# IRVLab/so_dso_place_recognition

Measured on AMD Instinct MI355X. Metric: queries/sec over 100k-signature DB (SC 20x60, z-score fusion, top-1), higher is better.
Workload: dtype f16x2 (fp32 carried as f16 hi + lo, fp32 accumulate); binary intensity channel: one f16 product per term, rounded to its exact integer count; 1 GPU; sc_match_100k; db_signatures=100000, descriptor=SC 20x60 x 2 channels, mask_width=0, k=1, db_rows_per_gpu=100000

## Files before the change

### so_dso_place_recognition_amd/csrc/sc_pack.hip

```cpp
#include <cstdlib>
#include <cstring>

#include "kernels.hpp"

namespace pr {
namespace {

constexpr int SC_PACK_FEW = 8;

template <typename T>
__global__ __launch_bounds__(256) void sc_pack_kernel(const T* __restrict__ sig, int rows, int role,
                                                       float* __restrict__ packed, int groups,
                                                       const double* __restrict__ tw, int* __restrict__ flags,
                                                       int* __restrict__ bad) {
  __shared__ double x[1200];
  __shared__ double red[256];
  __shared__ double tws[120];
  const int tid = threadIdx.x;
  const int row = blockIdx.x >> 1, ch = blockIdx.x & 1;
  const T* src = sig + (size_t)row * 2400 + ch * 1200;
  double part = 0.0;
  for (int i = tid; i < 1200; i += 256) {
    double v = (double)src[i];
    x[i] = v;
    part += v * v;
  }
  if (tid < 120) tws[tid] = tw[tid];
  red[tid] = part;
  __syncthreads();
  for (int s = 128; s > 0; s >>= 1) {
    if (tid < s) red[tid] += red[tid + s];
    __syncthreads();
  }
  const double nr = sqrt(red[0]);
  const bool isbad = !(nr > 0.0) || !(nr < __builtin_inf());
  if (tid == 0) { bad[2 * row + ch] = isbad ? (1 << ch) : 0; if (isbad) atomicOr(flags, 1); }
  for (int i = tid; i < 1200; i += 256) x[i] = isbad ? 0.0 : x[i] / nr;
  __syncthreads();
  const double scale = 0.12909944487358055;
  for (int o = tid; o < SC_NF * 40; o += 256) {
    const int f = o / 40, rem = o - f * 40, ring = rem >> 1, im = rem & 1;
    double acc = 0.0;
    int t = 0;
    for (int s = 0; s < 60; s++) {
      const double w = im ? -tws[60 + t] : tws[t];
      acc += x[s * 20 + ring] * w;
      t += f;
      if (t >= 60) t -= 60;
    }
    const float val = (float)(acc * scale);
    const int s4 = ring >> 2, k = ring & 3;
    size_t dst;
    if (role == 0) {
      const int g = row >> 3, e = row & 7;
      const int lane = (k << 4) | (im << 3) | e;
      dst = ((size_t)ch * groups + g) * SC_QIMG + (size_t)sc_fpos(f) * 320 + s4 * 64 + lane;
    } else {
      const int g = row >> 4, j = row & 15;
      const int lane = (k << 4) | j;
      const size_t base = ((size_t)ch * groups + g) * SC_DIMG + (size_t)sc_fpos(f) * SC_DSTEP;
      dst = (s4 < 4) ? base + im * 256 + lane * 4 + s4 : base + 512 + lane * 2 + im;
    }
    packed[dst] = val;
  }
}


template <typename T>
__global__ __launch_bounds__(320) void sc_pack_h_kernel(const T* __restrict__ sig, int rows, int role,
                                                         unsigned short* __restrict__ packed, int groups,
                                                         const double* __restrict__ tw, int* __restrict__ flags,
                                                         int* __restrict__ bad) {
  __shared__ double x[1200];
  __shared__ double red[320];
  __shared__ double tws[120];
  const int tid = threadIdx.x;
  const int row = blockIdx.x >> 1, ch = blockIdx.x & 1;
  const T* src = sig + (size_t)row * 2400 + ch * 1200;
  double part = 0.0;
  for (int i = tid; i < 1200; i += 320) {
    double v = (double)src[i];
    x[i] = v;
    part += v * v;
  }
  if (tid < 120) tws[tid] = tw[tid];
  red[tid] = part;
  __syncthreads();
  if (tid < 64) red[tid] += red[tid + 256];
  __syncthreads();
  for (int s = 128; s > 0; s >>= 1) {
    if (tid < s) red[tid] += red[tid + s];
    __syncthreads();
  }
  const double nr = sqrt(red[0]);
  const bool isbad = !(nr > 0.0) || !(nr < __builtin_inf());
  if (tid == 0) { bad[2 * row + ch] = isbad ? (1 << ch) : 0; if (isbad) atomicOr(flags, 1); }
  for (int i = tid; i < 1200; i += 320) x[i] = isbad ? 0.0 : x[i] / nr;
  __syncthreads();
  const double scale = 0.12909944487358055 * (role == 0 ? 256.0 : 128.0);
  {
    const int o = tid;
    const int f = o / 20, ring = o - f * 20;
    double ce = 0.0, co = 0.0, se = 0.0, so = 0.0;
    int t = 0;
#pragma unroll 3
    for (int s2 = 0; s2 < 60; s2 += 2) {
      const double x0 = x[s2 * 20 + ring];
      ce += x0 * tws[t];
      se += x0 * tws[60 + t];
      t += f; if (t >= 60) t -= 60;
      const double x1 = x[(s2 + 1) * 20 + ring];
      co += x1 * tws[t];
      so += x1 * tws[60 + t];
      t += f; if (t >= 60) t -= 60;
    }
    auto put = [&](double val, int ff, int im) {
      const _Float16 hi = (_Float16)val;
      const _Float16 lo = (_Float16)(val - (double)hi);
      size_t bh, bl;
      if (role == 0) {
        const int g = row >> 3, rr = (im << 3) | (row & 7);
        const size_t base = ((size_t)ch * groups + g) * SCH_QIMG + (size_t)ff * SCH_QBLK + rr * 80 + (rr >= 8 ? 8 : 0);
        bh = base + ring * 2;
        bl = base + sch_qlo_byte(ring);
      } else {
        const int g = row >> 4, j = row & 15;
        const size_t base = ((size_t)ch * groups + g) * SCH_DIMG + (size_t)ff * SCH_DFREQ + (size_t)im * 2 * SCH_DTILE +
                            (((ring >> 3) << 4) | j) * 16 + (ring & 7) * 2;
        bh = base;
        bl = base + SCH_DTILE;
        if (ring >= 16) packed[(bl + 8) >> 1] = __builtin_bit_cast(unsigned short, hi);
      }
      packed[bh >> 1] = __builtin_bit_cast(unsigned short, hi);
      packed[bl >> 1] = __builtin_bit_cast(unsigned short, lo);
    };
    put((ce + co) * scale, f, 0);
    put(-(se + so) * scale, f, 1);
    if (f != 15) {
      put((ce - co) * scale, 30 - f, 0);
      put((se - so) * scale, 30 - f, 1);
    }
  }
}

template <typename T, int ROLE, bool LO>
__global__ __launch_bounds__(320) void sc_pack_h_col_kernel(const T* __restrict__ sig, int rows,
                                                             unsigned short* __restrict__ packed, int groups,
                                                             const double* __restrict__ tw, int* __restrict__ flags,
                                                             int* __restrict__ bad, float* __restrict__ binfo, int* __restrict__ bstat) {
  constexpr int SL = ROLE == 0 ? (LO ? SCH_QBLK : SCF_QBLK) : (LO ? SCH_DFREQ : SCF_DFREQ);
  constexpr int NG = ROLE == 0 ? 2 : 1;
  constexpr int IMGB = ROLE == 0 ? (LO ? SCH_QIMG : SCF_QIMG) : (LO ? SCH_DIMG : SCF_DIMG);
  constexpr int QROW = LO ? 80 : 40;
  __shared__ __attribute__((aligned(16))) char img[NG * 8 * SL];
  __shared__ double part[16 * 20];
  __shared__ int bnz[LO ? 320 : 1];
  __shared__ float epart[LO ? 320 : 1];
  const int tid = threadIdx.x, lrow = tid / 20, ring = tid - 20 * lrow;
  const int xcd = blockIdx.x & 7, idx = blockIdx.x >> 3;
  const int fb = idx & 3, ch = (idx >> 2) & 1, blk = (idx >> 3) * 8 + xcd;
  if (blk * 16 >= rows) return;
  const int row = blk * 16 + lrow;
  const bool valid = row < rows;
  for (int i = tid; i < NG * 8 * SL / 8; i += 320) reinterpret_cast<unsigned long long*>(img)[i] = 0ull;
  const T* src = sig + (size_t)(valid ? row : 0) * 2400 + ch * 1200 + ring;
  double ce[4] = {0, 0, 0, 0}, co[4] = {0, 0, 0, 0}, se[4] = {0, 0, 0, 0}, so[4] = {0, 0, 0, 0};
  double nsq = 0.0;
  const bool do_eps = LO && binfo != nullptr && ch == 1, do_bin = do_eps && fb == 0;
  int nz = 0;
  double vmn = __builtin_inf(), vmx = -__builtin_inf();
  float e2 = 0.f;
  const double* twc = tw + 120 + (size_t)fb * 60 * 8;
#ifndef SCP_AHEAD
#define SCP_AHEAD 2
#endif
  constexpr int XR = SCP_AHEAD + 1;
  static_assert(15 % XR == 0, "the ring size must divide the 15 rounds");
  T xq[XR][4];
#pragma unroll
  for (int r = 0; r < SCP_AHEAD; r++)
#pragma unroll
    for (int k = 0; k < 4; k++) xq[r][k] = src[(r * 4 + k) * 20];
#pragma unroll XR
  for (int it = 0; it < 15; it++) {
    if (it + SCP_AHEAD < 15) {
#pragma unroll
      for (int k = 0; k < 4; k++) xq[(it + SCP_AHEAD) % XR][k] = src[((it + SCP_AHEAD) * 4 + k) * 20];
    }
    int tz = 0;
    asm volatile("" : "+s"(tz), "+v"(ce[0]), "+v"(ce[1]), "+v"(ce[2]), "+v"(ce[3]), "+v"(co[0]), "+v"(co[1]), "+v"(co[2]), "+v"(co[3]),
                      "+v"(se[0]), "+v"(se[1]), "+v"(se[2]), "+v"(se[3]), "+v"(so[0]), "+v"(so[1]), "+v"(so[2]), "+v"(so[3]));
    const double* tp = twc + it * 32 + tz;
#pragma unroll
    for (int h = 0; h < 2; h++) {
      const double x0 = (double)xq[it % XR][2 * h], x1 = (double)xq[it % XR][2 * h + 1];
      nsq += x0 * x0;
      nsq += x1 * x1;
      if (do_bin) {
        if (x0 != 0.0) { nz++; vmn = fmin(vmn, x0); vmx = fmax(vmx, x0); }
        if (x1 != 0.0) { nz++; vmn = fmin(vmn, x1); vmx = fmax(vmx, x1); }
      }
#pragma unroll
      for (int j = 0; j < 4; j++) {
        ce[j] += x0 * tp[h * 16 + 2 * j];
        se[j] += x0 * tp[h * 16 + 2 * j + 1];
        co[j] += x1 * tp[h * 16 + 8 + 2 * j];
        so[j] += x1 * tp[h * 16 + 8 + 2 * j + 1];
      }
    }
  }
  part[tid] = nsq;
  if (LO && do_bin) bnz[tid] = (nz == 0 || (vmn == vmx && vmn > 0.0)) ? nz : -1;
  __syncthreads();
  double n2 = 0.0;
#pragma unroll
  for (int r = 0; r < 20; r++) n2 += part[lrow * 20 + r];
  const double nr = sqrt(n2);
  const bool isbad = !(nr > 0.0) || !(nr < __builtin_inf());
  if (valid && ring == 0 && fb == 0) { bad[2 * row + ch] = isbad ? (1 << ch) : 0; if (isbad) atomicOr(flags, 1); }
  const int srow = blk * 16 + tid;
  bool sbad = true;
  if (LO && do_eps && tid < 16) {
    double n2t = 0.0;
#pragma unroll
    for (int r = 0; r < 20; r++) n2t += part[tid * 20 + r];
    const double nrt = sqrt(n2t);
    sbad = srow >= rows || !(nrt > 0.0) || !(nrt < __builtin_inf());
  }
  if (LO && do_bin) {
    __syncthreads();
    part[tid] = vmx;
    __syncthreads();
    if (tid < 16) {
      int ones = 0;
      bool binary = true;
      double a = -__builtin_inf();
      for (int r = 0; r < 20; r++) {
        const int c = bnz[tid * 20 + r];
        const double v = part[tid * 20 + r];
        if (c < 0) binary = false;
        if (c > 0) { ones += c; if (a == -__builtin_inf()) a = v; else if (v != a) binary = false; }
      }
      binary = binary && ones > 0;
      float s1 = 1.f, rs = 1.f;
      if (!sbad && binary) { s1 = (float)sqrt((double)ones); rs = (float)(1.0 / sqrt((double)ones)); }
      if (srow < rows) { binfo[2 * srow] = s1; binfo[2 * srow + 1] = rs; }
      int mo = (!sbad && binary) ? ones : 0, nb = (!sbad && !binary) ? 1 : 0;
#pragma unroll
      for (int o = 8; o > 0; o >>= 1) { mo = max(mo, __shfl_xor(mo, o)); nb |= __shfl_xor(nb, o); }
      if (tid == 0) { bstat[SC_BSTAT_INTS + 6 * blk] = nb; bstat[SC_BSTAT_INTS + 6 * blk + 1] = mo; }
    }
  }
  const double sc = isbad ? 0.0 : 0.12909944487358055 * (ROLE == 0 ? 256.0 : 128.0) / nr;
  auto put = [&](double val, int slice, int im) {
    if (isbad) val = 0.0;
    float vf = (float)val;
    asm volatile("" : "+v"(vf));
    const _Float16 hi = (_Float16)vf;
    float rf = (float)(val - (double)hi);
    asm volatile("" : "+v"(rf));
    const _Float16 lo = (_Float16)rf;
    int bh, bl;
    if (ROLE == 0) {
      const int rr = (im << 3) | (lrow & 7);
      bh = ((lrow >> 3) * 8 + slice) * SL + rr * QROW + ((LO && rr >= 8) ? 8 : 0) + ring * 2;
      bl = bh - ring * 2 + sch_qlo_byte(ring);
    } else {
      bh = slice * SL + im * (LO ? 2 : 1) * SCH_DTILE + (((ring >> 3) << 4) | lrow) * 16 + (ring & 7) * 2;
      bl = bh + SCH_DTILE;
      if (LO && ring >= 16) *reinterpret_cast<_Float16*>(img + bl + 8) = hi;
    }
    *reinterpret_cast<_Float16*>(img + bh) = hi;
    if (LO) *reinterpret_cast<_Float16*>(img + bl) = lo;
    if (LO) {
      const bool edge = (fb == 0 && (slice & 3) == 0);
      e2 = __builtin_fmaf(edge ? rf : 2.f * rf, rf, e2);
    }
  };
  if (valid) {
#pragma unroll
    for (int j = 0; j < 4; j++) {
      put((ce[j] + co[j]) * sc, j, 0);
      put(-(se[j] + so[j]) * sc, j, 1);
      if (4 * fb + j != 15) {
        put((ce[j] - co[j]) * sc, 4 + j, 0);
        put((se[j] - so[j]) * sc, 4 + j, 1);
      }
    }
  }
  if (LO && do_eps) epart[tid] = e2;
  __syncthreads();
  if (LO && do_eps && tid < 16) {
    float e = 0.f;
    for (int r = 0; r < 20; r++) e += epart[tid * 20 + r];
    if (sbad) e = 0.f;
#pragma unroll
    for (int o = 8; o > 0; o >>= 1) e = fmaxf(e, __shfl_xor(e, o));
    const int eb = __float_as_int(e * (ROLE == 0 ? 0x1p-16f : 0x1p-14f) * (1.f + 0x1p-10f));
    if (tid == 0) bstat[SC_BSTAT_INTS + 6 * blk + 2 + fb] = eb;
  }
  constexpr int W = SL / 8;
  for (int i = tid; i < NG * 8 * W; i += 320) {
    const int sl = i / W, wd = i - sl * W, gg = sl >> 3, k = sl & 7;
    const int f = k < 4 ? 4 * fb + k : 30 - 4 * fb - (k - 4);
    if (k >= 4 && f == 15) continue;
    const int g = NG * blk + gg;
    if (g >= groups) continue;
    reinterpret_cast<unsigned long long*>(reinterpret_cast<char*>(packed) + ((size_t)ch * groups + g) * IMGB + (size_t)f * SL)[wd] =
        reinterpret_cast<const unsigned long long*>(img)[i];
  }
}

__device__ __forceinline__ double wave_sum(double v) {
#pragma unroll
  for (int o = 32; o > 0; o >>= 1) v += __shfl_xor(v, o);
  return v;
}
template <typename T, int ROLE, bool LO>
__global__ __launch_bounds__(320) void sc_pack_h_few_kernel(const T* __restrict__ sig, int rows, unsigned short* __restrict__ packed, int groups,
                                                             const double* __restrict__ tw, int* __restrict__ flags, int* __restrict__ bad,
                                                             float* __restrict__ binfo, int* __restrict__ bstat,
                                                             int row0 ) {
  constexpr int SL = ROLE == 0 ? (LO ? SCH_QBLK : SCF_QBLK) : (LO ? SCH_DFREQ : SCF_DFREQ);
  constexpr int IMGB = ROLE == 0 ? (LO ? SCH_QIMG : SCF_QIMG) : (LO ? SCH_DIMG : SCF_DIMG);
  constexpr int QROW = LO ? 80 : 40;
  __shared__ double x[1200];
  __shared__ double tws[120];
  __shared__ double part[20];
  __shared__ double wred[5][3];
  const int tid = threadIdx.x, f = tid / 20, ring = tid - 20 * f;
  const int row = row0 + (blockIdx.x >> 1), ch = blockIdx.x & 1;
  const T* src = sig + (size_t)(blockIdx.x >> 1) * 2400 + ch * 1200;
  const bool do_bin = LO && binfo != nullptr && ch == 1;
  double bz = 0.0, bmn_ = __builtin_inf(), bmx_ = -__builtin_inf();
  for (int i = tid; i < 1200; i += 320) {
    const double v = (double)src[i];
    x[i] = v;
    if (do_bin && v != 0.0) { bz += 1.0; bmn_ = fmin(bmn_, v); bmx_ = fmax(bmx_, v); }
  }
  if (do_bin) {
#pragma unroll
    for (int o = 32; o > 0; o >>= 1) { bz += __shfl_xor(bz, o); bmn_ = fmin(bmn_, __shfl_xor(bmn_, o)); bmx_ = fmax(bmx_, __shfl_xor(bmx_, o)); }
    if ((tid & 63) == 0) { wred[tid >> 6][0] = bz; wred[tid >> 6][1] = bmn_; wred[tid >> 6][2] = bmx_; }
  }
  if (tid < 120) tws[tid] = tw[tid];
  __syncthreads();
  double ce = 0.0, co = 0.0, se = 0.0, so = 0.0, nsq = 0.0;
  int t = 0;
#pragma unroll 1
  for (int s2 = 0; s2 < 60; s2 += 2) {
    const double x0 = x[s2 * 20 + ring], x1 = x[(s2 + 1) * 20 + ring];
    nsq += x0 * x0;
    nsq += x1 * x1;
    ce += x0 * tws[t];
    se += x0 * tws[60 + t];
    t += f; if (t >= 60) t -= 60;
    co += x1 * tws[t];
    so += x1 * tws[60 + t];
    t += f; if (t >= 60) t -= 60;
  }
  if (f == 0) part[ring] = nsq;
  __syncthreads();
  double n2 = 0.0;
#pragma unroll
  for (int r = 0; r < 20; r++) n2 += part[r];
  const double nr = sqrt(n2);
  const bool isbad = !(nr > 0.0) || !(nr < __builtin_inf());
  if (tid == 0) { bad[2 * row + ch] = isbad ? (1 << ch) : 0; if (isbad) atomicOr(flags, 1); }
  if (do_bin && tid == 0) {
    double ones = 0.0, mn = __builtin_inf(), mx = -__builtin_inf();
    for (int w5 = 0; w5 < 5; w5++) { ones += wred[w5][0]; mn = fmin(mn, wred[w5][1]); mx = fmax(mx, wred[w5][2]); }
    const bool binary = ones > 0.0 && mn == mx && mn > 0.0;
    float s = 1.f, rs = 1.f;
    if (!isbad && binary) { s = (float)sqrt(ones); rs = (float)(1.0 / sqrt(ones)); atomicMax(bstat + 1, (int)ones); }
    if (!isbad && !binary) atomicOr(bstat, 1);
    binfo[2 * row] = s; binfo[2 * row + 1] = rs;
  }
  const double sc = isbad ? 0.0 : 0.12909944487358055 * (ROLE == 0 ? 256.0 : 128.0) / nr;
  char* out = reinterpret_cast<char*>(packed);
  double e2 = 0.0;
  auto put = [&](double val, int ff, int im) {
    if (isbad) val = 0.0;
    float vf = (float)val;
    asm volatile("" : "+v"(vf));
    const _Float16 hi = (_Float16)vf;
    float rf = (float)(val - (double)hi);
    asm volatile("" : "+v"(rf));
    const _Float16 lo = (_Float16)rf;
    if (do_bin) {
      const double r = (val - (double)hi) * (ROLE == 0 ? 0x1p-8 : 0x1p-7);
      e2 += ((ff == 0 || ff == 30) ? 1.0 : 2.0) * r * r;
    }
    size_t bh;
    if (ROLE == 0) {
      const int g = row >> 3, rr = (im << 3) | (row & 7);
      bh = ((size_t)ch * groups + g) * IMGB + (size_t)ff * SL + rr * QROW + ((LO && rr >= 8) ? 8 : 0) + ring * 2;
      *reinterpret_cast<_Float16*>(out + bh) = hi;
      if (LO) *reinterpret_cast<_Float16*>(out + bh - ring * 2 + sch_qlo_byte(ring)) = lo;
    } else {
      const int g = row >> 4, j = row & 15;
      bh = ((size_t)ch * groups + g) * IMGB + (size_t)ff * SL + (size_t)im * (LO ? 2 : 1) * SCH_DTILE + (((ring >> 3) << 4) | j) * 16 + (ring & 7) * 2;
      *reinterpret_cast<_Float16*>(out + bh) = hi;
      if (LO) *reinterpret_cast<_Float16*>(out + bh + SCH_DTILE) = lo;
      if (LO && ring >= 16) *reinterpret_cast<_Float16*>(out + bh + SCH_DTILE + 8) = hi;
    }
  };
  put((ce + co) * sc, f, 0);
  put(-(se + so) * sc, f, 1);
  if (f != 15) {
    put((ce - co) * sc, 30 - f, 0);
    put((se - so) * sc, 30 - f, 1);
  }
  if (do_bin) {
    e2 = wave_sum(e2);
    __syncthreads();
    if ((tid & 63) == 0) wred[tid >> 6][0] = e2;
    __syncthreads();
    if (tid == 0 && !isbad) {
      double e = 0.0;
      for (int w5 = 0; w5 < 5; w5++) e += wred[w5][0];
      atomicMax(bstat + 2, __float_as_int((float)(e * (1.0 + 0x1p-20))));
    }
  }
}

__global__ __launch_bounds__(256) void sc_bstat_finalize_kernel(int* __restrict__ bstat, int nblk) {
  __shared__ int red[6][256];
  int v[6] = {0, 0, 0, 0, 0, 0};
  for (int b = threadIdx.x; b < nblk; b += 256) {
    const int* w = bstat + SC_BSTAT_INTS + 6 * b;
    v[0] |= w[0];
#pragma unroll
    for (int i = 1; i < 6; i++) v[i] = max(v[i], w[i]);
  }
#pragma unroll
  for (int i = 0; i < 6; i++) red[i][threadIdx.x] = v[i];
  __syncthreads();
  for (int s2 = 128; s2 > 0; s2 >>= 1) {
    if ((int)threadIdx.x < s2) {
      red[0][threadIdx.x] |= red[0][threadIdx.x + s2];
#pragma unroll
      for (int i = 1; i < 6; i++) red[i][threadIdx.x] = max(red[i][threadIdx.x], red[i][threadIdx.x + s2]);
    }
    __syncthreads();
  }
  if (threadIdx.x < 6) bstat[threadIdx.x] = red[threadIdx.x][0];
}

template <typename T, int ROLE, bool LO = true>
void launch_pack_col(hipStream_t st, const T* sig, int rows, unsigned short* packed, int groups, const double* tw, int* flags, int* bad,
                     float* binfo = nullptr, int* bstat = nullptr) {
  if (rows <= SC_PACK_FEW) {
    hipLaunchKernelGGL((sc_pack_h_few_kernel<T, ROLE, LO>), dim3((unsigned)rows * 2), dim3(320), 0, st, sig, rows, packed, groups, tw, flags, bad,
                       binfo, bstat, 0);
    return;
  }
  hipLaunchKernelGGL((sc_pack_h_col_kernel<T, ROLE, LO>), dim3((unsigned)(((rows + 15) / 16 + 7) / 8) * 64), dim3(320), 0, st, sig, rows, packed,
                     groups, tw, flags, bad, binfo, bstat);
  if (LO && bstat) hipLaunchKernelGGL(sc_bstat_finalize_kernel, dim3(1), dim3(256), 0, st, bstat, (rows + 15) / 16);
}

__global__ __launch_bounds__(256) void zero_ints_kernel(int* __restrict__ p, int n) {
  const int i = blockIdx.x * 256 + threadIdx.x;
  if (i < n) p[i] = 0;
}

__global__ __launch_bounds__(256) void fill_ints_kernel(int* __restrict__ p, int n, int v) {
  const int i = blockIdx.x * 256 + threadIdx.x;
  if (i < n) p[i] = v;
}

}

void launch_zero_ints(hipStream_t st, int* p, int n) {
  if (n > 0) hipLaunchKernelGGL(zero_ints_kernel, dim3((n + 255) / 256), dim3(256), 0, st, p, n);
}
void launch_fill_ints(hipStream_t st, int* p, int n, int v) {
  if (n > 0) hipLaunchKernelGGL(fill_ints_kernel, dim3((n + 255) / 256), dim3(256), 0, st, p, n, v);
}

void launch_sc_pack_h(hipStream_t st, const void* sig, int dtype, int rows, int role, void* packed, int groups,
                      const double* twiddle, int* flags, int* bad, int single, float* binfo, int* bstat) {
  if (rows <= 0) return;
  if (single) {
    if (dtype == 0 && role == 0) launch_pack_col<double, 0, false>(st, (const double*)sig, rows, (unsigned short*)packed, groups, twiddle, flags, bad);
    else if (dtype == 0) launch_pack_col<double, 1, false>(st, (const double*)sig, rows, (unsigned short*)packed, groups, twiddle, flags, bad);
    else if (role == 0) launch_pack_col<float, 0, false>(st, (const float*)sig, rows, (unsigned short*)packed, groups, twiddle, flags, bad);
    else launch_pack_col<float, 1, false>(st, (const float*)sig, rows, (unsigned short*)packed, groups, twiddle, flags, bad);
    return;
  }
  static const bool valu = getenv("PR_SC_PACK") && !strcmp(getenv("PR_SC_PACK"), "valu");
  if (valu && bstat) hipLaunchKernelGGL(fill_ints_kernel, dim3(1), dim3(256), 0, st, bstat, 1, 1);
  if (valu && dtype == 0)
    hipLaunchKernelGGL(sc_pack_h_kernel<double>, dim3(rows * 2), dim3(320), 0, st, (const double*)sig, rows, role,
                       (unsigned short*)packed, groups, twiddle, flags, bad);
  else if (valu)
    hipLaunchKernelGGL(sc_pack_h_kernel<float>, dim3(rows * 2), dim3(320), 0, st, (const float*)sig, rows, role,
                       (unsigned short*)packed, groups, twiddle, flags, bad);
  else if (dtype == 0 && role == 0) launch_pack_col<double, 0>(st, (const double*)sig, rows, (unsigned short*)packed, groups, twiddle, flags, bad, binfo, bstat);
  else if (dtype == 0) launch_pack_col<double, 1>(st, (const double*)sig, rows, (unsigned short*)packed, groups, twiddle, flags, bad, binfo, bstat);
  else if (role == 0) launch_pack_col<float, 0>(st, (const float*)sig, rows, (unsigned short*)packed, groups, twiddle, flags, bad, binfo, bstat);
  else launch_pack_col<float, 1>(st, (const float*)sig, rows, (unsigned short*)packed, groups, twiddle, flags, bad, binfo, bstat);
}

void launch_sc_pack_h_rows(hipStream_t st, const void* sig, int dtype, int rows, int row0, void* packed, int groups, const double* twiddle,
                           int* flags, int* bad, int single, float* binfo, int* bstat) {
  if (rows <= 0) return;
  unsigned short* pk = (unsigned short*)packed;
  const dim3 grid((unsigned)rows * 2), blk(320);
  if (single) {
    if (dtype == 0) hipLaunchKernelGGL((sc_pack_h_few_kernel<double, 1, false>), grid, blk, 0, st, (const double*)sig, rows, pk, groups, twiddle, flags, bad, nullptr, nullptr, row0);
    else hipLaunchKernelGGL((sc_pack_h_few_kernel<float, 1, false>), grid, blk, 0, st, (const float*)sig, rows, pk, groups, twiddle, flags, bad, nullptr, nullptr, row0);
  } else {
    if (dtype == 0) hipLaunchKernelGGL((sc_pack_h_few_kernel<double, 1, true>), grid, blk, 0, st, (const double*)sig, rows, pk, groups, twiddle, flags, bad, binfo, bstat, row0);
    else hipLaunchKernelGGL((sc_pack_h_few_kernel<float, 1, true>), grid, blk, 0, st, (const float*)sig, rows, pk, groups, twiddle, flags, bad, binfo, bstat, row0);
  }
}

void launch_sc_pack(hipStream_t st, const void* sig, int dtype, int rows, int role, float* packed, int groups,
                    const double* twiddle, int* flags, int* bad) {
  if (rows <= 0) return;
  if (dtype == 0)
    hipLaunchKernelGGL(sc_pack_kernel<double>, dim3(rows * 2), dim3(256), 0, st, (const double*)sig, rows, role,
                       packed, groups, twiddle, flags, bad);
  else
    hipLaunchKernelGGL(sc_pack_kernel<float>, dim3(rows * 2), dim3(256), 0, st, (const float*)sig, rows, role,
                       packed, groups, twiddle, flags, bad);
}

}
```

Baseline: 138,600 queries/s.

## Replace direct DFT in SC packing with factored real FFT-60

The column pack kernel now computes each 60-point ring DFT with a factored real FFT (radix-4 by 15, with the 15-point part split as 3 by 5) held in registers per thread, instead of a twiddle-table direct DFT where each thread produced one frequency. One block now handles all 31 frequencies of 16 rows and writes them out in four staged slices, so the grid shrinks and the per-element multiply-adds drop from O(N^2) to roughly O(N log N). The few-row kernel also uses the FFT, on 20 threads. The old kernel stays behind a PR_SC_PACK=dense env switch. In exchange, the roughly 60-double register arrays raise register pressure, and the rounding differs from the direct sum, which could change the hi/lo split bits.

```diff
diff --git a/so_dso_place_recognition_amd/csrc/sc_pack.hip b/so_dso_place_recognition_amd/csrc/sc_pack.hip
--- a/so_dso_place_recognition_amd/csrc/sc_pack.hip
+++ b/so_dso_place_recognition_amd/csrc/sc_pack.hip
@@ -144,7 +144,7 @@
 }
 
 template <typename T, int ROLE, bool LO>
-__global__ __launch_bounds__(320) void sc_pack_h_col_kernel(const T* __restrict__ sig, int rows,
+__global__ __launch_bounds__(320) void sc_pack_h_col_dense_kernel(const T* __restrict__ sig, int rows,
                                                              unsigned short* __restrict__ packed, int groups,
                                                              const double* __restrict__ tw, int* __restrict__ flags,
                                                              int* __restrict__ bad, float* __restrict__ binfo, int* __restrict__ bstat) {
@@ -311,6 +311,251 @@
   }
 }
 
+struct ScR5 { double a0, a1, b1, a2, b2; };
+__device__ __forceinline__ ScR5 sc_rdft5(double r0, double r1, double r2, double r3, double r4) {
+#pragma clang fp contract(off)
+  constexpr double C1 = 0.30901699437494742410, C2 = -0.80901699437494742410;
+  constexpr double S1 = 0.95105651629515357212, S2 = 0.58778525229247312917;
+  const double s1 = r1 + r4, s2 = r2 + r3, d1 = r1 - r4, d2 = r2 - r3;
+  ScR5 o;
+  o.a0 = r0 + (s1 + s2);
+  o.a1 = __builtin_fma(C2, s2, __builtin_fma(C1, s1, r0));
+  o.a2 = __builtin_fma(C1, s2, __builtin_fma(C2, s1, r0));
+  o.b1 = __builtin_fma(S2, d2, S1 * d1);
+  o.b2 = __builtin_fma(-S1, d2, S2 * d1);
+  return o;
+}
+template <int ST>
+__device__ __forceinline__ void sc_rdft15(const double* z, double* re, double* im) {
+#pragma clang fp contract(off)
+  constexpr double S3 = 0.86602540378443864676;
+  double r0[5], p[5], q[5];
+#pragma unroll
+  for (int b = 0; b < 5; b++) {
+    const double z0 = z[ST * ((3 * b) % 15)], z1 = z[ST * ((5 + 3 * b) % 15)], z2 = z[ST * ((10 + 3 * b) % 15)];
+    const double s = z1 + z2;
+    r0[b] = z0 + s;
+    p[b] = __builtin_fma(-0.5, s, z0);
+    q[b] = S3 * (z2 - z1);
+  }
+  const ScR5 v0 = sc_rdft5(r0[0], r0[1], r0[2], r0[3], r0[4]);
+  const ScR5 vp = sc_rdft5(p[0], p[1], p[2], p[3], p[4]);
+  const ScR5 vq = sc_rdft5(q[0], q[1], q[2], q[3], q[4]);
+  re[0] = v0.a0;          im[0] = 0.0;
+  re[1] = vp.a1 + vq.b1;  im[1] = vq.a1 - vp.b1;
+  re[2] = vp.a2 - vq.b2;  im[2] = -(vq.a2 + vp.b2);
+  re[3] = v0.a2;          im[3] = v0.b2;
+  re[4] = vp.a1 - vq.b1;  im[4] = vq.a1 + vp.b1;
+  re[5] = vp.a0;          im[5] = -vq.a0;
+  re[6] = v0.a1;          im[6] = -v0.b1;
+  re[7] = vp.a2 + vq.b2;  im[7] = vq.a2 - vp.b2;
+}
+__device__ __forceinline__ void sc_rdft60(const double* x, double* re, double* im) {
+#pragma clang fp contract(off)
+  double z[60];
+#pragma unroll
+  for (int m = 0; m < 15; m++) {
+    const double a = x[(4 * m) % 60], b = x[(15 + 4 * m) % 60], c = x[(30 + 4 * m) % 60], d = x[(45 + 4 * m) % 60];
+    const double ac = a + c, bd = b + d;
+    z[4 * m] = ac + bd;
+    z[4 * m + 1] = ac - bd;
+    z[4 * m + 2] = a - c;
+    z[4 * m + 3] = b - d;
+  }
+  double u0r[8], u0i[8], u2r[8], u2i[8], ar[8], ai[8], br[8], bi[8];
+  sc_rdft15<4>(z, u0r, u0i);
+  sc_rdft15<4>(z + 1, u2r, u2i);
+  sc_rdft15<4>(z + 2, ar, ai);
+  sc_rdft15<4>(z + 3, br, bi);
+#pragma unroll
+  for (int k = 0; k <= 30; k++) {
+    const int k15 = k % 15, kk = k15 <= 7 ? k15 : 15 - k15;
+    const double cj = k15 <= 7 ? 1.0 : -1.0;
+    switch (k & 3) {
+      case 0: re[k] = u0r[kk]; im[k] = cj * u0i[kk]; break;
+      case 2: re[k] = u2r[kk]; im[k] = cj * u2i[kk]; break;
+      case 1: re[k] = ar[kk] + cj * bi[kk]; im[k] = cj * ai[kk] - br[kk]; break;
+      default: re[k] = ar[kk] - cj * bi[kk]; im[k] = cj * ai[kk] + br[kk]; break;
+    }
+  }
+}
+
+__device__ __forceinline__ double sc_row_sq(const double* x) {
+  double nsq = 0.0;
+#pragma unroll
+  for (int s = 0; s < 60; s++) nsq = __builtin_fma(x[s], x[s], nsq);
+  return nsq;
+}
+__device__ __forceinline__ void sc_split(double spec, double sc, bool zero, _Float16& hi, _Float16& lo, double& res) {
+#pragma clang fp contract(off)
+  double val = spec * sc;
+  if (zero) val = 0.0;
+  float vf = (float)val;
+  asm volatile("" : "+v"(vf));
+  hi = (_Float16)vf;
+  res = val - (double)hi;
+  float rf = (float)res;
+  asm volatile("" : "+v"(rf));
+  lo = (_Float16)rf;
+}
+
+template <typename T, int ROLE, bool LO>
+__global__ __launch_bounds__(320) __attribute__((amdgpu_waves_per_eu(3))) void sc_pack_h_col_kernel(const T* __restrict__ sig, int rows,
+                                                             unsigned short* __restrict__ packed, int groups, int* __restrict__ flags,
+                                                             int* __restrict__ bad, float* __restrict__ binfo, int* __restrict__ bstat) {
+  constexpr int SL = ROLE == 0 ? (LO ? SCH_QBLK : SCF_QBLK) : (LO ? SCH_DFREQ : SCF_DFREQ);
+  constexpr int NG = ROLE == 0 ? 2 : 1;
+  constexpr int IMGB = ROLE == 0 ? (LO ? SCH_QIMG : SCF_QIMG) : (LO ? SCH_DIMG : SCF_DIMG);
+  constexpr int QROW = LO ? 80 : 40;
+  __shared__ __attribute__((aligned(16))) char img[NG * 8 * SL];
+  __shared__ double part[16 * 20];
+  __shared__ int bnz[LO ? 320 : 1];
+  __shared__ float epart[LO ? 4 * 320 : 1];
+  const int tid = threadIdx.x, lrow = tid / 20, ring = tid - 20 * lrow;
+  const int ch = blockIdx.x & 1, blk = blockIdx.x >> 1;
+  const int row = blk * 16 + lrow;
+  const bool valid = row < rows;
+  for (int i = tid; i < NG * 8 * SL / 8; i += 320) reinterpret_cast<unsigned long long*>(img)[i] = 0ull;
+  const T* src = sig + (size_t)(valid ? row : 0) * 2400 + ch * 1200 + ring;
+  const bool do_eps = LO && binfo != nullptr && ch == 1;
+  double x[60];
+#pragma unroll
+  for (int s = 0; s < 60; s++) x[s] = (double)src[s * 20];
+  const double nsq = sc_row_sq(x);
+  int nz = 0;
+  double vmn = __builtin_inf(), vmx = -__builtin_inf();
+  if (do_eps) {
+#pragma unroll
+    for (int s = 0; s < 60; s++)
+      if (x[s] != 0.0) { nz++; vmn = fmin(vmn, x[s]); vmx = fmax(vmx, x[s]); }
+  }
+  part[tid] = nsq;
+  if (LO && do_eps) bnz[tid] = (nz == 0 || (vmn == vmx && vmn > 0.0)) ? nz : -1;
+  __syncthreads();
+  double n2 = 0.0;
+#pragma unroll
+  for (int r = 0; r < 20; r++) n2 += part[lrow * 20 + r];
+  const double nr = sqrt(n2);
+  const bool isbad = !(nr > 0.0) || !(nr < __builtin_inf());
+  if (valid && ring == 0) { bad[2 * row + ch] = isbad ? (1 << ch) : 0; if (isbad) atomicOr(flags, 1); }
+  const int srow = blk * 16 + tid;
+  bool sbad = true;
+  if (LO && do_eps && tid < 16) {
+    double n2t = 0.0;
+#pragma unroll
+    for (int r = 0; r < 20; r++) n2t += part[tid * 20 + r];
+    const double nrt = sqrt(n2t);
+    sbad = srow >= rows || !(nrt > 0.0) || !(nrt < __builtin_inf());
+  }
+  if (LO && do_eps) {
+    __syncthreads();
+    part[tid] = vmx;
+    __syncthreads();
+    if (tid < 16) {
+      int ones = 0;
+      bool binary = true;
+      double a = -__builtin_inf();
+      for (int r = 0; r < 20; r++) {
+        const int c = bnz[tid * 20 + r];
+        const double v = part[tid * 20 + r];
+        if (c < 0) binary = false;
+        if (c > 0) { ones += c; if (a == -__builtin_inf()) a = v; else if (v != a) binary = false; }
+      }
+      binary = binary && ones > 0;
+      float s1 = 1.f, rs = 1.f;
+      if (!sbad && binary) { s1 = (float)sqrt((double)ones); rs = (float)(1.0 / sqrt((double)ones)); }
+      if (srow < rows) { binfo[2 * srow] = s1; binfo[2 * srow + 1] = rs; }
+      int mo = (!sbad && binary) ? ones : 0, nb = (!sbad && !binary) ? 1 : 0;
+#pragma unroll
+      for (int o = 8; o > 0; o >>= 1) { mo = max(mo, __shfl_xor(mo, o)); nb |= __shfl_xor(nb, o); }
+      if (tid == 0) { bstat[SC_BSTAT_INTS + 6 * blk] = nb; bstat[SC_BSTAT_INTS + 6 * blk + 1] = mo; }
+    }
+  }
+  const double sc = isbad ? 0.0 : 0.12909944487358055 * (ROLE == 0 ? 256.0 : 128.0) / nr;
+  float e2[4] = {0.f, 0.f, 0.f, 0.f};
+  unsigned pk[62];
+  {
+    double re[31], im[31];
+    sc_rdft60(x, re, im);
+    auto split = [&](double spec, int fb, bool edge) -> unsigned {
+      _Float16 hi, lo;
+      double res;
+      sc_split(spec, sc, isbad || !valid, hi, lo, res);
+      if (LO) {
+        const float rf = (float)res;
+        e2[fb] = __builtin_fmaf(edge ? rf : 2.f * rf, rf, e2[fb]);
+      }
+      return (unsigned)__builtin_bit_cast(unsigned short, hi) | ((unsigned)__builtin_bit_cast(unsigned short, lo) << 16);
+    };
+#pragma unroll
+    for (int f = 0; f <= 15; f++) {
+      pk[2 * f] = split(re[f], f >> 2, f == 0);
+      pk[2 * f + 1] = split(im[f], f >> 2, f == 0);
+      if (f != 15) {
+        pk[2 * (30 - f)] = split(re[30 - f], f >> 2, f == 0);
+        pk[2 * (30 - f) + 1] = split(im[30 - f], f >> 2, f == 0);
+      }
+    }
+  }
+  auto put = [&](unsigned hl, int slice, int im_) {
+    const _Float16 hi = __builtin_bit_cast(_Float16, (unsigned short)(hl & 0xffffu)), lo = __builtin_bit_cast(_Float16, (unsigned short)(hl >> 16));
+    int bh, bl;
+    if (ROLE == 0) {
+      const int rr = (im_ << 3) | (lrow & 7);
+      bh = ((lrow >> 3) * 8 + slice) * SL + rr * QROW + ((LO && rr >= 8) ? 8 : 0) + ring * 2;
+      bl = bh - ring * 2 + sch_qlo_byte(ring);
+    } else {
+      bh = slice * SL + im_ * (LO ? 2 : 1) * SCH_DTILE + (((ring >> 3) << 4) | lrow) * 16 + (ring & 7) * 2;
+      bl = bh + SCH_DTILE;
+      if (LO && ring >= 16) *reinterpret_cast<_Float16*>(img + bl + 8) = hi;
+    }
+    *reinterpret_cast<_Float16*>(img + bh) = hi;
+    if (LO) *reinterpret_cast<_Float16*>(img + bl) = lo;
+  };
+  constexpr int W = SL / 8;
+#pragma unroll
+  for (int fb = 0; fb < 4; fb++) {
+    if (fb) __syncthreads();
+#pragma unroll
+    for (int j = 0; j < 4; j++) {
+      const int f = 4 * fb + j;
+      put(pk[2 * f], j, 0);
+      put(pk[2 * f + 1], j, 1);
+      if (f != 15) {
+        put(pk[2 * (30 - f)], 4 + j, 0);
+        put(pk[2 * (30 - f) + 1], 4 + j, 1);
+      }
+    }
+    __syncthreads();
+    for (int i = tid; i < NG * 8 * W; i += 320) {
+      const int sl = i / W, wd = i - sl * W, gg = sl >> 3, k = sl & 7;
+      const int f = k < 4 ? 4 * fb + k : 30 - 4 * fb - (k - 4);
+      if (k >= 4 && f == 15) continue;
+      const int g = NG * blk + gg;
+      if (g >= groups) continue;
+      reinterpret_cast<unsigned long long*>(reinterpret_cast<char*>(packed) + ((size_t)ch * groups + g) * IMGB + (size_t)f * SL)[wd] =
+          reinterpret_cast<const unsigned long long*>(img)[i];
+    }
+  }
+  if (LO && do_eps) {
+#pragma unroll
+    for (int fb = 0; fb < 4; fb++) epart[fb * 320 + tid] = e2[fb];
+    __syncthreads();
+    if (tid < 16) {
+#pragma unroll
+      for (int fb = 0; fb < 4; fb++) {
+        float e = 0.f;
+        for (int r = 0; r < 20; r++) e += epart[fb * 320 + tid * 20 + r];
+        if (sbad) e = 0.f;
+#pragma unroll
+        for (int o = 8; o > 0; o >>= 1) e = fmaxf(e, __shfl_xor(e, o));
+        const int eb = __float_as_int(e * (ROLE == 0 ? 0x1p-16f : 0x1p-14f) * (1.f + 0x1p-10f));
+        if (tid == 0) bstat[SC_BSTAT_INTS + 6 * blk + 2 + fb] = eb;
+      }
+    }
+  }
+}
+
 __device__ __forceinline__ double wave_sum(double v) {
 #pragma unroll
   for (int o = 32; o > 0; o >>= 1) v += __shfl_xor(v, o);
@@ -318,14 +563,14 @@
 }
 template <typename T, int ROLE, bool LO>
 __global__ __launch_bounds__(320) void sc_pack_h_few_kernel(const T* __restrict__ sig, int rows, unsigned short* __restrict__ packed, int groups,
-                                                             const double* __restrict__ tw, int* __restrict__ flags, int* __restrict__ bad,
+                                                             int* __restrict__ flags, int* __restrict__ bad,
                                                              float* __restrict__ binfo, int* __restrict__ bstat,
                                                              int row0 ) {
   constexpr int SL = ROLE == 0 ? (LO ? SCH_QBLK : SCF_QBLK) : (LO ? SCH_DFREQ : SCF_DFREQ);
   constexpr int IMGB = ROLE == 0 ? (LO ? SCH_QIMG : SCF_QIMG) : (LO ? SCH_DIMG : SCF_DIMG);
   constexpr int QROW = LO ? 80 : 40;
   __shared__ double x[1200];
-  __shared__ double tws[120];
+  __shared__ double spec[62][20];
   __shared__ double part[20];
   __shared__ double wred[5][3];
   const int tid = threadIdx.x, f = tid / 20, ring = tid - 20 * f;
@@ -343,23 +588,16 @@
     for (int o = 32; o > 0; o >>= 1) { bz += __shfl_xor(bz, o); bmn_ = fmin(bmn_, __shfl_xor(bmn_, o)); bmx_ = fmax(bmx_, __shfl_xor(bmx_, o)); }
     if ((tid & 63) == 0) { wred[tid >> 6][0] = bz; wred[tid >> 6][1] = bmn_; wred[tid >> 6][2] = bmx_; }
   }
-  if (tid < 120) tws[tid] = tw[tid];
-  __syncthreads();
-  double ce = 0.0, co = 0.0, se = 0.0, so = 0.0, nsq = 0.0;
-  int t = 0;
-#pragma unroll 1
-  for (int s2 = 0; s2 < 60; s2 += 2) {
-    const double x0 = x[s2 * 20 + ring], x1 = x[(s2 + 1) * 20 + ring];
-    nsq += x0 * x0;
-    nsq += x1 * x1;
-    ce += x0 * tws[t];
-    se += x0 * tws[60 + t];
-    t += f; if (t >= 60) t -= 60;
-    co += x1 * tws[t];
-    so += x1 * tws[60 + t];
-    t += f; if (t >= 60) t -= 60;
-  }
-  if (f == 0) part[ring] = nsq;
+  __syncthreads();
+  if (tid < 20) {
+    double xr[60], re[31], im[31];
+#pragma unroll
+    for (int s = 0; s < 60; s++) xr[s] = x[s * 20 + tid];
+    part[tid] = sc_row_sq(xr);
+    sc_rdft60(xr, re, im);
+#pragma unroll
+    for (int k = 0; k <= 30; k++) { spec[2 * k][tid] = re[k]; spec[2 * k + 1][tid] = im[k]; }
+  }
   __syncthreads();
   double n2 = 0.0;
 #pragma unroll
@@ -379,16 +617,12 @@
   const double sc = isbad ? 0.0 : 0.12909944487358055 * (ROLE == 0 ? 256.0 : 128.0) / nr;
   char* out = reinterpret_cast<char*>(packed);
   double e2 = 0.0;
-  auto put = [&](double val, int ff, int im) {
-    if (isbad) val = 0.0;
-    float vf = (float)val;
-    asm volatile("" : "+v"(vf));
-    const _Float16 hi = (_Float16)vf;
-    float rf = (float)(val - (double)hi);
-    asm volatile("" : "+v"(rf));
-    const _Float16 lo = (_Float16)rf;
+  auto put = [&](int ff, int im) {
+    _Float16 hi, lo;
+    double res;
+    sc_split(spec[2 * ff + im][ring], sc, isbad, hi, lo, res);
     if (do_bin) {
-      const double r = (val - (double)hi) * (ROLE == 0 ? 0x1p-8 : 0x1p-7);
+      const double r = res * (ROLE == 0 ? 0x1p-8 : 0x1p-7);
       e2 += ((ff == 0 || ff == 30) ? 1.0 : 2.0) * r * r;
     }
     size_t bh;
@@ -405,11 +639,11 @@
       if (LO && ring >= 16) *reinterpret_cast<_Float16*>(out + bh + SCH_DTILE + 8) = hi;
     }
   };
-  put((ce + co) * sc, f, 0);
-  put(-(se + so) * sc, f, 1);
+  put(f, 0);
+  put(f, 1);
   if (f != 15) {
-    put((ce - co) * sc, 30 - f, 0);
-    put((se - so) * sc, 30 - f, 1);
+    put(30 - f, 0);
+    put(30 - f, 1);
   }
   if (do_bin) {
     e2 = wave_sum(e2);
@@ -451,12 +685,18 @@
 void launch_pack_col(hipStream_t st, const T* sig, int rows, unsigned short* packed, int groups, const double* tw, int* flags, int* bad,
                      float* binfo = nullptr, int* bstat = nullptr) {
   if (rows <= SC_PACK_FEW) {
-    hipLaunchKernelGGL((sc_pack_h_few_kernel<T, ROLE, LO>), dim3((unsigned)rows * 2), dim3(320), 0, st, sig, rows, packed, groups, tw, flags, bad,
+    hipLaunchKernelGGL((sc_pack_h_few_kernel<T, ROLE, LO>), dim3((unsigned)rows * 2), dim3(320), 0, st, sig, rows, packed, groups, flags, bad,
                        binfo, bstat, 0);
     return;
   }
-  hipLaunchKernelGGL((sc_pack_h_col_kernel<T, ROLE, LO>), dim3((unsigned)(((rows + 15) / 16 + 7) / 8) * 64), dim3(320), 0, st, sig, rows, packed,
-                     groups, tw, flags, bad, binfo, bstat);
+  const char* mode = getenv("PR_SC_PACK");
+  const bool dense = mode && !strcmp(mode, "dense");
+  if (dense)
+    hipLaunchKernelGGL((sc_pack_h_col_dense_kernel<T, ROLE, LO>), dim3((unsigned)(((rows + 15) / 16 + 7) / 8) * 64), dim3(320), 0, st, sig, rows,
+                       packed, groups, tw, flags, bad, binfo, bstat);
+  else
+    hipLaunchKernelGGL((sc_pack_h_col_kernel<T, ROLE, LO>), dim3((unsigned)((rows + 15) / 16) * 2), dim3(320), 0, st, sig, rows, packed, groups,
+                       flags, bad, binfo, bstat);
   if (LO && bstat) hipLaunchKernelGGL(sc_bstat_finalize_kernel, dim3(1), dim3(256), 0, st, bstat, (rows + 15) / 16);
 }
 
@@ -509,11 +749,11 @@
   unsigned short* pk = (unsigned short*)packed;
   const dim3 grid((unsigned)rows * 2), blk(320);
   if (single) {
-    if (dtype == 0) hipLaunchKernelGGL((sc_pack_h_few_kernel<double, 1, false>), grid, blk, 0, st, (const double*)sig, rows, pk, groups, twiddle, flags, bad, nullptr, nullptr, row0);
-    else hipLaunchKernelGGL((sc_pack_h_few_kernel<float, 1, false>), grid, blk, 0, st, (const float*)sig, rows, pk, groups, twiddle, flags, bad, nullptr, nullptr, row0);
+    if (dtype == 0) hipLaunchKernelGGL((sc_pack_h_few_kernel<double, 1, false>), grid, blk, 0, st, (const double*)sig, rows, pk, groups, flags, bad, nullptr, nullptr, row0);
+    else hipLaunchKernelGGL((sc_pack_h_few_kernel<float, 1, false>), grid, blk, 0, st, (const float*)sig, rows, pk, groups, flags, bad, nullptr, nullptr, row0);
   } else {
-    if (dtype == 0) hipLaunchKernelGGL((sc_pack_h_few_kernel<double, 1, true>), grid, blk, 0, st, (const double*)sig, rows, pk, groups, twiddle, flags, bad, binfo, bstat, row0);
-    else hipLaunchKernelGGL((sc_pack_h_few_kernel<float, 1, true>), grid, blk, 0, st, (const float*)sig, rows, pk, groups, twiddle, flags, bad, binfo, bstat, row0);
+    if (dtype == 0) hipLaunchKernelGGL((sc_pack_h_few_kernel<double, 1, true>), grid, blk, 0, st, (const double*)sig, rows, pk, groups, flags, bad, binfo, bstat, row0);
+    else hipLaunchKernelGGL((sc_pack_h_few_kernel<float, 1, true>), grid, blk, 0, st, (const float*)sig, rows, pk, groups, flags, bad, binfo, bstat, row0);
   }
 }
 
```

Result: no change. 137,800 queries/s (-0.6%).
